# joesound212985/Deepfake-Detection-using-CLIP-Based-SigLIP-2-Vision-Transformers

Hardware: AMD Instinct MI355X
Metric: images/sec (train fwd+bwd) SigLIP-2-so400m@384 bf16 (higher is better)
Workload: dtype bf16; 1 GPU; so400m-patch14-384 encoder+pool-head train fwd+bwd, 384x384, per-GPU batch 128, seeded random weights; global_batch=128, parallelism=dp1

## Files before the change

deepfake-detection-using-clip-based-siglip-2-vision-transformers_amd/csrc/encoder.hip:

```cpp
#include <hip/hip_runtime.h>
#include <string.h>

#include <algorithm>
#include <new>
#include <vector>

#include "kernels.h"
#include "siglip_hip.h"

using namespace sgl;

namespace {

inline size_t align256(size_t x) { return (x + 255) & ~(size_t)255; }
inline char* at(void* base, size_t off) { return reinterpret_cast<char*>(base) + off; }
inline const char* at(const void* base, size_t off) { return reinterpret_cast<const char*>(base) + off; }
inline bool mfma16(int dt) { return dt == DT_BF16 || dt == DT_F16; }
inline int round_up(int x, int m) { return (x + m - 1) / m * m; }

struct Bump {
  size_t off = 0;
  size_t take(size_t bytes) {
    const size_t o = off;
    off += align256(bytes);
    return o;
  }
};

struct ShadowLayer {
  size_t wqkv, wqkv_t, wo, wo_t, w1, w1_t, w2, w2_t, bqkv, b1;
  size_t wqkv_s, wo_s, w1_s, w2_s;
};

}

struct sgl_ctx {
  sgl_config cfg;
  int D, I, Ip, L, H, dh, DP, P, K0, Kp, g0, dt;
  size_t es;
  int split = 0;
  int mx = 0;
  int Dp = 0;
  int recompute = 0;
  int last_hip = 0;
  size_t sh_wpatch = 0;
  std::vector<ShadowLayer> sh_layers;
  size_t sh_hwkv = 0, sh_hwkv_t = 0, sh_hwo = 0, sh_hwo_t = 0, sh_hw1 = 0, sh_hw1_t = 0, sh_hw2 = 0, sh_hw2_t = 0,
         sh_hb1 = 0;
  size_t sh_total = 0;
};

namespace {

constexpr int kMaxLayers = 128;

constexpr size_t kSplitWsBytes = (size_t)256 * 256 * 256 * 4;

inline size_t head_bytes(const sgl_ctx* c, int B, int N) { return (size_t)B * c->H * N * c->DP * c->es; }

struct Layout {
  int B = 0, gh = 0, gw = 0, N = 0, M = 0;
  bool train = false;
  size_t a_im2col = 0, a_pos = 0;
  size_t a_layer0 = 0, a_layer_stride = 0;
  size_t r_stats1 = 0, r_h1 = 0, r_qkv = 0, r_attn = 0, r_lse = 0, r_xmid = 0, r_stats2 = 0, r_h2 = 0, r_u = 0, r_a = 0,
         r_attq = 0;
  size_t a_pstats = 0, a_lastlp = 0, a_kvh = 0, a_qp = 0, a_probs = 0, a_ao = 0, a_h0 = 0, a_hstats = 0, a_hl = 0, a_hu = 0,
         a_ha = 0;
  size_t a_spa = 0, a_spb = 0, w_spa = 0, w_spb = 0;
  size_t act_total = 0;
  size_t w_dx = 0, w_g = 0, w_du = 0, w_dh = 0, w_dqkv = 0, w_delta = 0, w_splitws = 0, w_lnpart = 0, w_cspart = 0,
         w_dlast = 0, w_gsum = 0, w_csum = 0;
  size_t w_hg = 0, w_hdu = 0, w_hdh = 0, w_hdao = 0, w_hdqpart = 0, w_hdqp = 0, w_hdh0 = 0;
  size_t ws_bwd_total = 0;
  size_t saved_total = 0, ws_total = 0, ws_act_off = 0;
  bool rc = false;
  size_t w_blk = 0;

  Layout() = default;
  Layout(const sgl_ctx* c, int B_, int Himg, int Wimg, bool train_) {
    B = B_;
    train = train_;
    rc = train && c->recompute;
    gh = Himg / c->P;
    gw = Wimg / c->P;
    N = gh * gw;
    M = B * N;
    const size_t es = c->es, D = c->D, Ip = c->Ip, Mz = (size_t)M;
    Bump a;
    a_im2col = a.take(Mz * c->Kp * es);
    a_pos = a.take((size_t)N * D * 4);
    Bump r;
    const size_t Dp = c->Dp;
    const bool mx = c->mx;
    r_stats1 = r.take(Mz * 2 * 4);
    r_h1 = r.take(mx ? Mz * Dp + Mz * Dp / 32 : Mz * D * es);
    r_qkv = r.take(3 * head_bytes(c, B, N));
    r_attn = r.take(Mz * D * es);
    r_lse = r.take((size_t)B * c->H * N * 4);
    r_xmid = r.take(Mz * D * 4);
    r_stats2 = r.take(Mz * 2 * 4);
    r_h2 = r.take(mx ? Mz * Dp + Mz * Dp / 32 : Mz * D * es);
    r_u = r.take(mx ? 0 : Mz * Ip * es);
    r_a = r.take(mx ? Mz * Ip + Mz * Ip / 32 : Mz * Ip * es);
    r_attq = r.take(mx ? Mz * Dp + Mz * Dp / 32 : 0);
    a_layer_stride = (train && !rc) ? r.off : 0;
    a_layer0 = a.take(rc ? 0 : train ? r.off * (size_t)c->L : r.off);
    a_pstats = a.take(Mz * 2 * 4);
    a_lastlp = a.take(Mz * D * es);
// ... 1303 lines not shown
```

deepfake-detection-using-clip-based-siglip-2-vision-transformers_amd/csrc/gemm_bf16.hip:

```cpp
#include <stdlib.h>

#include "common.hip.h"
#include "epilogue.hip.h"
#include "kernels.h"

namespace sgl {

constexpr int G_BM = 128, G_BN = 128, G_BK = 64;
constexpr int G_STAGE = (G_BM + G_BN) * G_BK * 2;
constexpr int G_CT_LD = 132;
constexpr int G_LDS = (2 * G_STAGE > G_BM * G_CT_LD * 4) ? 2 * G_STAGE : G_BM * G_CT_LD * 4;

__device__ __forceinline__ u32x4 ldg128(__amdgpu_buffer_rsrc_t r, uint32_t voff) {
  return __builtin_amdgcn_raw_buffer_load_b128(r, voff, 0, 0);
}

template <int EPI, typename TOut>
__device__ __forceinline__ void store_tile(char* smem, f32x4 (&acc)[4][4], int wr, int wc, int lane, int t, int m0,
                                           int n0, int M, int N, const EpiParams& p) {
  float* ct = reinterpret_cast<float*>(smem);
  __syncthreads();
  const int g = lane >> 4, c16 = lane & 15;
#pragma unroll
  for (int i = 0; i < 4; ++i)
// ... 217 lines not shown
#pragma unroll
      for (int i = 0; i < 4; ++i)
#pragma unroll
        for (int j = 0; j < 4; ++j)
          acc[i][j] = mfma_16x16x32(af[i], bfr[j], acc[i][j]);
    }
    if (kt + 1 < nk) store_stage(cur ^ 1);
    __syncthreads();
  }
  EpiParams pq = p;
  if (p.split_stride) pq.out = reinterpret_cast<float*>(p.out) + (size_t)blockIdx.y * p.split_stride;
  store_tile<EPI_F32, float>(smem, acc, wr, wc, lane, t, n1_0, n2_0, N1, N2, pq);
}

template <int EPI, typename TOut, typename TIn>
static hipError_t launch_nt(const TIn* A, int lda, const TIn* B, int ldb, int M, int N, int K, const EpiParams& p,
                            hipStream_t s) {
  const hipError_t e = set_max_dynamic_lds_once<&gemm_nt_kernel<EPI, TOut, TIn>>(G_LDS);
  if (e != hipSuccess) return e;
  const int tiles = ((M + G_BM - 1) / G_BM) * ((N + G_BN - 1) / G_BN);
  hipLaunchKernelGGL((gemm_nt_kernel<EPI, TOut, TIn>), dim3(tiles), dim3(256), G_LDS, s, A, lda, B, ldb, M, N, K, p);
  return hipGetLastError();
}

template <typename TIn>
static hipError_t gemm_nt_mfma(const void* A, int lda, const void* B, int ldb, int M, int N, int K, int epi,
                               int out_dtype, const EpiParams& p, hipStream_t s) {
  if (M == 0 || N == 0) return hipSuccess;
  if ((lda % 8) || (ldb % 8) || (K % 8) || K <= 0) return hipErrorInvalidValue;
  if (epi != EPI_F32 && (N % 8)) return hipErrorInvalidValue;
  if ((size_t)M * lda * 2 >= (1ull << 32) || (size_t)N * ldb * 2 >= (1ull << 32)) return hipErrorInvalidValue;
  if (M >= 2048 && N >= 256) {
    static const int tile_env = getenv("SGL_NT_TILE") ? atoi(getenv("SGL_NT_TILE")) : 0;
    const bool can384 = epi == EPI_STORE || epi == EPI_RES_F32;
    const bool pays384 = N % 192 == 0 && N % 256 != 0 && (epi == EPI_STORE || K >= 2048);
    const bool want384 = tile_env == 384 || (tile_env != 256 && pays384);
    if (can384 && want384) return gemm_nt384<TIn>(A, lda, B, ldb, M, N, K, epi, out_dtype, p, s);
    return gemm_nt256<TIn>(A, lda, B, ldb, M, N, K, epi, out_dtype, p, s);
  }
  return dispatch_epilogue<TIn>(epi, out_dtype, [&](auto tag) {
    using T = decltype(tag);
    return launch_nt<T::epi, typename T::out, TIn>((const TIn*)A, lda, (const TIn*)B, ldb, M, N, K, p, s);
  });
}
hipError_t gemm_nt_bf16(const void* A, int lda, const void* B, int ldb, int M, int N, int K, int epi, int out_dtype,
                        const EpiParams& p, hipStream_t s) {
  return gemm_nt_mfma<bf16>(A, lda, B, ldb, M, N, K, epi, out_dtype, p, s);
}
hipError_t gemm_nt_f16(const void* A, int lda, const void* B, int ldb, int M, int N, int K, int epi, int out_dtype,
                       const EpiParams& p, hipStream_t s) {
  return gemm_nt_mfma<f16>(A, lda, B, ldb, M, N, K, epi, out_dtype, p, s);
}

template <typename Launch>
static hipError_t tn_split_k(int Mred, int N1, int N2, int splits, const EpiParams& p_, hipStream_t s, float* split_ws,
                             size_t split_ws_bytes, Launch&& launch) {
  EpiParams p = p_;
  float* out = reinterpret_cast<float*>(p.out);
  if (splits < 1) splits = 1;
  int m_per = (Mred + splits - 1) / splits;
  m_per = ((m_per + G_BK - 1) / G_BK) * G_BK;
  splits = (Mred + m_per - 1) / m_per;
  if (splits > 1) {
    const size_t slab = (size_t)N1 * N2;
    if (split_ws && (size_t)splits * slab * sizeof(float) <= split_ws_bytes && p.alpha == 1.0f && !p.bias &&
        (N2 % 4 == 0) && (p.ldo % 4 == 0) && ((((uintptr_t)out) | ((uintptr_t)split_ws)) & 15) == 0) {
      EpiParams q = p;
      q.out = split_ws;
      q.ldo = N2;
      q.accumulate = 0;
      q.atomic = 0;
      q.split_stride = slab;
      const hipError_t e = launch(m_per, splits, q);
      if (e != hipSuccess) return e;
      return reduce_splits(split_ws, splits, slab, N1, N2, out, p.ldo, p.accumulate, s);
    }
    if (!p.accumulate) {
      const hipError_t e = hipMemset2DAsync(out, (size_t)p.ldo * sizeof(float), 0, (size_t)N2 * sizeof(float), N1, s);
      if (e != hipSuccess) return e;
    }
    p.atomic = 1;
  }
  return launch(m_per, splits, p);
}

template <typename TIn>
static hipError_t gemm_tn_mfma(const void* A, int lda, const void* B, int ldb, int Mred, int N1, int N2, int splits,
                               const EpiParams& p, hipStream_t s, float* split_ws, size_t split_ws_bytes) {
  if (N1 == 0 || N2 == 0) return hipSuccess;
  if ((lda % 8) || (ldb % 8)) return hipErrorInvalidValue;
  if ((size_t)Mred * lda * 2 >= (1ull << 32) || (size_t)Mred * ldb * 2 >= (1ull << 32)) return hipErrorInvalidValue;
  if (Mred <= 0) {
    if (!p.accumulate)
      return hipMemset2DAsync(p.out, (size_t)p.ldo * sizeof(float), 0, (size_t)N2 * sizeof(float), N1, s);
    return hipSuccess;
  }
  if (N1 >= 512 && N2 >= 512 && Mred >= 2048) {
    const int tiles = ((N1 + 255) / 256) * ((N2 + 255) / 256);
    int sp = 256 / tiles;
    if (sp < 1) sp = 1;
    const int max_sp = Mred / 1024 > 0 ? Mred / 1024 : 1;
    if (sp > max_sp) sp = max_sp;
    return tn_split_k(Mred, N1, N2, sp, p, s, split_ws, split_ws_bytes, [&](int m_per, int nsplit, const EpiParams& q) {
      return gemm_tn256<TIn>(A, lda, B, ldb, Mred, N1, N2, m_per, nsplit, q, s);
    });
  }
  return tn_split_k(Mred, N1, N2, splits, p, s, split_ws, split_ws_bytes, [&](int m_per, int nsplit, const EpiParams& q) {
    const hipError_t e = set_max_dynamic_lds_once<&gemm_tn_kernel<TIn>>(G_LDS);
    if (e != hipSuccess) return e;
    const int tiles = ((N1 + G_BM - 1) / G_BM) * ((N2 + G_BN - 1) / G_BN);
    hipLaunchKernelGGL(gemm_tn_kernel<TIn>, dim3(tiles, nsplit), dim3(256), G_LDS, s, (const TIn*)A, lda, (const TIn*)B,
                       ldb, Mred, N1, N2, m_per, q);
    return hipGetLastError();
  });
}
hipError_t gemm_tn_bf16(const void* A, int lda, const void* B, int ldb, int Mred, int N1, int N2, int splits,
                        const EpiParams& p, hipStream_t s, float* split_ws, size_t split_ws_bytes) {
  return gemm_tn_mfma<bf16>(A, lda, B, ldb, Mred, N1, N2, splits, p, s, split_ws, split_ws_bytes);
}
hipError_t gemm_tn_f16(const void* A, int lda, const void* B, int ldb, int Mred, int N1, int N2, int splits,
                       const EpiParams& p, hipStream_t s, float* split_ws, size_t split_ws_bytes) {
  return gemm_tn_mfma<f16>(A, lda, B, ldb, Mred, N1, N2, splits, p, s, split_ws, split_ws_bytes);
}

}
```

deepfake-detection-using-clip-based-siglip-2-vision-transformers_amd/csrc/gemm_bf16_v2.hip:

```cpp
#include <stdlib.h>
#ifdef SGL_TIMELINE
#include <stdio.h>
#include <string.h>
#endif

#include "common.hip.h"
#include "epilogue.hip.h"
#include "kernels.h"

namespace sgl {

constexpr int T_BK = 64;

template <int BM_, int BN_, int MI_, int MJ_>
struct NtTileShape {
  static constexpr int BM = BM_, BN = BN_, MI = MI_, MJ = MJ_;
  static constexpr int WM = 16 * MI, WN = 16 * MJ;
  static constexpr int NWR = BM / WM, NWC = BN / WN;
  static constexpr int OPA = BM * T_BK * 2;
  static constexpr int STAGE = (BM + BN) * T_BK * 2;
  static constexpr int LDS = 2 * STAGE;
  static constexpr int PA = BM / 128, PB = BN / 64, NI = 2 * PA + PB;
  static constexpr int CT_LD = BN + 4;
  static_assert(NWR * WM == BM && NWC * WN == BN && NWR * NWC == 8, "8 waves = 512 threads cover the tile");
  static_assert(MI % 2 == 0 && BM % 128 == 0 && BN % 64 == 0 && 64 % NWR == 0 && (64 / NWR) % 16 == 0, "halves, pieces, passes");
  static_assert(LDS <= 160 * 1024 && 64 * CT_LD * 4 <= LDS, "two stages, and the epilogue image, in 160 KiB of LDS");
};

struct NtTile256 : NtTileShape<256, 256, 8, 4> {
  static __device__ __forceinline__ int wr(int w) { return (w >> 1) & 1; }
  static __device__ __forceinline__ int wc(int w) { return (w & 1) + 2 * (w >> 2); }
  static __device__ __forceinline__ int b_row(int w, int q) {
    const int ul = 16 * w + 8 * (q & 1);
    return (ul >> 5) * 64 + (ul & 31) + 32 * (q >> 1);
  }
  static constexpr bool takes(int epi) { return true; }
};

struct NtTile384 : NtTileShape<384, 192, 6, 6> {
  static __device__ __forceinline__ int wr(int w) { return w & 3; }
  static __device__ __forceinline__ int wc(int w) { return w >> 2; }
  static __device__ __forceinline__ int b_row(int w, int q) { return 8 * (3 * w + q); }
  static constexpr bool takes(int epi) { return epi == EPI_STORE || epi == EPI_RES_F32; }
};

constexpr int gcd_of(int a, int b) { return b == 0 ? a : gcd_of(b, a % b); }

template <typename G, int EPI, typename TOut>
__device__ __forceinline__ void store_tile_pp(char* smem, f32x4 (&acc)[G::MI][G::MJ], int wr, int wc, int lane, int t,
                                              int m0, int n0, int M, int N, const EpiParams& p) {
  static_assert(G::takes(EPI), "this tile geometry is not dispatched with this epilogue");
  float* ct = reinterpret_cast<float*>(smem);
  const int g = lane >> 4, c16 = lane & 15;
  constexpr int NV = (sizeof(TOut) == 4) ? 4 : 8;
  constexpr int CT_LD = G::CT_LD;
  constexpr int CPR = G::BN / NV;
  constexpr int WR_ROWS = 64 / G::NWR;
  constexpr int BLK = WR_ROWS / 16;
  constexpr int NPASS = G::BM / 64;
  constexpr int QN = (64 * CPR) / 512;
  constexpr int P = CPR / gcd_of(CPR, 512);
  static_assert(NPASS * BLK == G::MI && (64 * CPR) % 512 == 0 && (512 * P) % CPR == 0, "staging image and chunk walk");
  auto grow_of = [&](int pass, int row) { return m0 + (row / WR_ROWS) * G::WM + pass * WR_ROWS + row % WR_ROWS; };
  constexpr bool HAS_BIAS = (EPI == EPI_BIAS_GELU || EPI == EPI_RES_F32 || EPI == EPI_QKV);
  int tcol[P], gcol[P];
  bool col_ok[P];
  float bias[P][NV];
  size_t qkv_c0[P];
  int qkv_pad[P];
#pragma unroll
  for (int h = 0; h < P; ++h) {
    tcol[h] = ((t + 512 * h) % CPR) * NV;
    gcol[h] = n0 + tcol[h];
    col_ok[h] = gcol[h] < N;
#pragma unroll
    for (int j = 0; j < NV; ++j) bias[h][j] = 0.f;
    if constexpr (HAS_BIAS) {
      if (col_ok[h]) Vec<float, NV>::ld(p.bias + gcol[h], bias[h]);
    }
    qkv_c0[h] = 0;
    qkv_pad[h] = 0;
    if constexpr (EPI == EPI_QKV) {
      const int dm = p.heads * p.head_dim;
      const int which = gcol[h] / dm;
      const int hc = gcol[h] - which * dm;
      const int hd = hc / p.head_dim;
      const int d = hc - hd * p.head_dim;
      qkv_c0[h] = ((size_t)which * p.batch * p.heads + hd) * (size_t)p.tokens * p.head_dim_pad + d;
      qkv_pad[h] = (d + NV == p.head_dim) ? (p.head_dim_pad - p.head_dim) / NV : 0;
    }
  }
  float csum[NV];
#pragma unroll
  for (int j = 0; j < NV; ++j) csum[j] = 0.f;
  using PreT = u32x4;
  constexpr bool HAS_PRE = (EPI == EPI_RES_F32 || EPI == EPI_GELU_BWD);
// ... 73 lines not shown
            for (int j = 0; j < NV; ++j) u[j] = (float)ub[j];
          } else {
            const f32x4 uf = __builtin_bit_cast(f32x4, pre[pass & 1][q]);
#pragma unroll
            for (int j = 0; j < NV; ++j) u[j] = uf[j];
          }
          epi_gelu_bwd<TOut, NV>(p, v, u, reinterpret_cast<TOut*>(p.out) + (size_t)grow * p.ldo + gcol[h]);
#pragma unroll
          for (int j = 0; j < NV; ++j) csum[j] += v[j];
        } else {
          epi_apply<EPI, TOut, NV>(p, grow, gcol[h], N, v);
        }
      }
    }
  }
  if constexpr (EPI == EPI_GELU_BWD) {
    static_assert(P == 1, "the bias-gradient fold needs one column set per thread");
    epi_colsum_fold<512, G::BN, NV>(ct, csum, t, m0, n0, N, p);
  }
}

__device__ __forceinline__ int unit_of_block(int bid, int per) { return (bid & 7) * per + (bid >> 3); }

__device__ __forceinline__ void tile_of_unit(int u, int tiles_m, int tiles_n, int& tile_m, int& tile_n, int bh = 8) {
  const int band = u / (bh * tiles_n);
  const int rows = (tiles_m - band * bh < bh) ? tiles_m - band * bh : bh;
  const int r = u - band * bh * tiles_n;
  tile_n = r / rows;
  tile_m = band * bh + (r - tile_n * rows);
}

__device__ __forceinline__ bool tile_of_local(int xcd, int v, int tiles_m, int tiles_n, int cgw, int& tm, int& tn) {
  const int r_lo = (xcd * tiles_m) >> 3, r_hi = ((xcd + 1) * tiles_m) >> 3;
  const int R = r_hi - r_lo;
  if (v >= R * tiles_n) return false;
  const int full = R * cgw;
  const int g = v / full, rem = v - g * full;
  const int w = (tiles_n - g * cgw < cgw) ? tiles_n - g * cgw : cgw;
  const int r = rem / w;
  tm = r_lo + r;
  tn = g * cgw + (rem - r * w);
  return true;
}

__device__ __forceinline__ void pp_dma16(u32x4 desc, uint32_t lds_addr, uint32_t voff) {
  asm volatile("s_mov_b32 m0, %0\n\ts_nop 0\n\tbuffer_load_dwordx4 %1, %2, 0 offen lds"
               :: "s"(lds_addr), "v"(voff), "s"(desc) : "memory");
}
__device__ __forceinline__ u32x4 pp_desc(const void* base, uint32_t bytes) {
  const uint64_t q = (uint64_t)base;
  u32x4 d = {(uint32_t)q, (uint32_t)(q >> 32) & 0xffffu, bytes, 0x00020000u};
  return d;
}
template <int NI>
__device__ __forceinline__ void pp_end_read() {
  asm volatile("s_waitcnt vmcnt(%0) lgkmcnt(0)" :: "n"(NI) : "memory");
  __builtin_amdgcn_sched_barrier(0);
  __builtin_amdgcn_s_barrier();
  __builtin_amdgcn_sched_barrier(0);
}
#define SGL_PP_END_MFMA()                 \
  do {                                    \
    __builtin_amdgcn_sched_barrier(0);    \
    __builtin_amdgcn_s_barrier();         \
    __builtin_amdgcn_sched_barrier(0);    \
  } while (0)

#ifdef SGL_TIMELINE
__device__ unsigned long long g_nt6_tl[4];
__device__ unsigned long long g_tn6_tl[12];
#define SGL_TL_STAMP(v) const unsigned long long v = __builtin_readcyclecounter()
#else
#define SGL_TL_STAMP(v)
#endif

template <typename G, int EPI, typename TOut, typename TIn>
__global__ __launch_bounds__(512, 2) void gemm_nt6_kernel(const TIn* __restrict__ A, int lda,
                                                          const TIn* __restrict__ B, int ldb, int M, int N, int K,
                                                          int tiles_m, int tiles_n, int band_h, EpiParams p) {
  extern __shared__ __attribute__((aligned(16))) char smem[];
  SGL_TL_STAMP(tl0);
  const int ntiles = tiles_m * tiles_n;
  int tile_m, tile_n;
  if (band_h < 0) {
    if (!tile_of_local(blockIdx.x & 7, blockIdx.x >> 3, tiles_m, tiles_n, -band_h, tile_m, tile_n)) return;
  } else {
    const int unit = unit_of_block(blockIdx.x, (ntiles + 7) >> 3);
    if (unit >= ntiles) return;
    tile_of_unit(unit, tiles_m, tiles_n, tile_m, tile_n, band_h);
  }
  constexpr int MI = G::MI, MJ = G::MJ, HI = MI / 2, PA = G::PA, PB = G::PB, NI = G::NI;
  const int t = threadIdx.x, lane = t & 63;
  const int w = __builtin_amdgcn_readfirstlane(t >> 6);
  const int wr = G::wr(w), wc = G::wc(w), grp = w >> 2;
  const int m0 = tile_m * G::BM, n0 = tile_n * G::BN;
  const int rows_a = (M - m0 < G::BM) ? M - m0 : G::BM;
  const int rows_b = (N - n0 < G::BN) ? N - n0 : G::BN;
  const u32x4 da = pp_desc(A + (size_t)m0 * lda, (uint32_t)(((size_t)(rows_a - 1) * lda + K) * 2));
  const u32x4 db = pp_desc(B + (size_t)n0 * ldb, (uint32_t)(((size_t)(rows_b - 1) * ldb + K) * 2));
  const uint32_t lds0 = (uint32_t)(size_t)((SGL_LDS char*)smem);

  enum { U_A0 = 0, U_B = 1, U_A1 = 2 };
  constexpr int PMAX = PA > PB ? PA : PB;
  const int drow = lane >> 3, dchunk = (lane & 7) ^ drow;
  uint32_t voff[3][PMAX], ldst[3][PMAX];
#pragma unroll
// ... 38 lines not shown
  lo_x8<TIn> fa[2 * HI], fb[2 * MJ];
  auto mfma_slot = [&](int i0) {
    if (active) {
      __builtin_amdgcn_s_setprio(1);
#pragma unroll
      for (int h = 0; h < 2; ++h)
#pragma unroll
        for (int i = 0; i < HI; ++i)
#pragma unroll
          for (int j = 0; j < MJ; ++j)
            acc[i0 + i][j] = mfma_16x16x32(fa[HI * h + i], fb[MJ * h + j], acc[i0 + i][j]);
      __builtin_amdgcn_s_setprio(0);
    }
    SGL_PP_END_MFMA();
  };
  for (int kt = 0; kt < nk; ++kt) {
    const char* base = smem + (kt & 1) * G::STAGE;
    const char* pa = base + fa_base;
    const char* pb = base + fb_base;
    if (active) {
#pragma unroll
      for (int f = 0; f < 2 * MJ; ++f) fb[f] = *reinterpret_cast<const lo_x8<TIn>*>(pb + (f % MJ) * 2048 + ((f / MJ) ? c1 : c0));
#pragma unroll
      for (int f = 0; f < 2 * HI; ++f) fa[f] = *reinterpret_cast<const lo_x8<TIn>*>(pa + (f % HI) * 2048 + ((f / HI) ? c1 : c0));
    }
    issue(U_A1, kt + 1);
    pp_end_read<NI>();
    mfma_slot(0);
    if (active) {
#pragma unroll
      for (int f = 0; f < 2 * HI; ++f) fa[f] = *reinterpret_cast<const lo_x8<TIn>*>(pa + (HI + f % HI) * 2048 + ((f / HI) ? c1 : c0));
    }
    issue(U_A0, kt + 2); issue(U_B, kt + 2);
    pp_end_read<NI>();
    mfma_slot(HI);
  }
  if (grp == 0) SGL_PP_END_MFMA();
  asm volatile("s_waitcnt vmcnt(0)" ::: "memory");
#ifdef SGL_TIMELINE
  if (p.atomic == 77) return;
#endif
  SGL_TL_STAMP(tl1);
  store_tile_pp<G, EPI, TOut>(smem, acc, wr, wc, lane, t, m0, n0, M, N, p);
#ifdef SGL_TIMELINE
  SGL_TL_STAMP(tl2);
  if (t == 0) {
    atomicAdd(&g_nt6_tl[0], tl1 - tl0);
    atomicAdd(&g_nt6_tl[1], tl2 - tl1);
    atomicAdd(&g_nt6_tl[2], 1ull);
  }
#endif
}

template <typename TIn>
__global__ __launch_bounds__(512, 2) void gemm_tn6_kernel(const TIn* __restrict__ A, int lda,
                                                          const TIn* __restrict__ B, int ldb, int Mred, int N1, int N2,
                                                          int m_per_split, int nsplits, int tiles_1, int tiles_2,
                                                          EpiParams p) {
  using G = NtTile256;
  extern __shared__ __attribute__((aligned(16))) char smem[];
  const int ntiles = tiles_1 * tiles_2;
  const int nunits = ntiles * nsplits;
  const int unit = unit_of_block(blockIdx.x, (nunits + 7) >> 3);
  if (unit >= nunits) return;
  const int split = unit / ntiles, trem = unit - split * ntiles;
  const int tile1 = trem / tiles_2, tile2 = trem - tile1 * tiles_2;
  const int t = threadIdx.x, lane = t & 63;
  const int w = __builtin_amdgcn_readfirstlane(t >> 6);
  const int wr = G::wr(w), wc = G::wc(w), grp = w >> 2;
  const int n1_0 = tile1 * G::BM, n2_0 = tile2 * G::BN;
  const int m_begin = split * m_per_split;
  const int m_end = (m_begin + m_per_split < Mred) ? m_begin + m_per_split : Mred;
  const int rows = m_end - m_begin;
  const u32x4 da = pp_desc(A + (size_t)m_begin * lda, (uint32_t)((size_t)rows * lda * 2));
  const u32x4 db = pp_desc(B + (size_t)m_begin * ldb, (uint32_t)((size_t)rows * ldb * 2));
  const uint32_t lds0 = (uint32_t)(size_t)((SGL_LDS char*)smem);

  const int dr2 = lane >> 5, dslot = lane & 31;
  uint32_t voff[4][2], ldst[4][2];
#pragma unroll
  for (int u = 0; u < 4; ++u)
#pragma unroll
    for (int q = 0; q < 2; ++q) {
      const int r0 = 32 * (u >> 1) + 4 * w + 2 * q;
      const int row = r0 + dr2;
      const int chunk = dslot ^ (2 * (row & 3) + 8 * ((row >> 3) & 1));
      const bool isA = (u & 1) == 0;
      const int col = (isA ? n1_0 : n2_0) + chunk * 8;
      const int lim = isA ? N1 : N2;
      const int ld = isA ? lda : ldb;
      voff[u][q] = (col < lim) ? (uint32_t)(row * ld + col) * 2u : SGL_OOB;
      ldst[u][q] = lds0 + (isA ? 0 : G::OPA) + (uint32_t)r0 * 512u;
    }
  auto issue = [&](int u, int kt) {
    const uint32_t r0 = (uint32_t)kt * T_BK;
    const uint32_t sb = (uint32_t)((kt & 1) * G::STAGE);
    const bool isA = (u & 1) == 0;
    const u32x4 d = isA ? da : db;
    const uint32_t adv = r0 * (uint32_t)(isA ? lda : ldb) * 2u;
#pragma unroll
    for (int q = 0; q < 2; ++q) pp_dma16(d, ldst[u][q] + sb, voff[u][q] == SGL_OOB ? SGL_OOB : voff[u][q] + adv);
  };

  const int fg = lane >> 4, fq = (lane >> 2) & 3, fp = lane & 3;
  const uint32_t swz = (uint32_t)(32 * fq + 128 * (fg & 1));
  const uint32_t frow = (uint32_t)((8 * fg + fq) * 512);
  const uint32_t fa_col = ((uint32_t)(wr * 256 + 8 * fp)) ^ swz;
  const uint32_t fb_col = ((uint32_t)(wc * 128 + 8 * fp)) ^ swz;
  const bool active = (n2_0 + wc * G::WN < N2) && (n1_0 + wr * G::WM < N1);

  f32x4 acc[G::MI][G::MJ];
#pragma unroll
  for (int i = 0; i < 8; ++i)
#pragma unroll
    for (int j = 0; j < 4; ++j) acc[i][j] = f32x4{0.f, 0.f, 0.f, 0.f};

  const int nk = (rows + T_BK - 1) / T_BK;
  issue(0, 0); issue(1, 0); issue(2, 0); issue(3, 0);
  issue(0, 1); issue(1, 1);
  pp_end_read<8>();
  if (grp == 1) SGL_PP_END_MFMA();

#define SGL_TR6(ptr) \
  __builtin_shufflevector(lds_read_tr16<TIn>(ptr), lds_read_tr16<TIn>((ptr) + 4 * 512), 0, 1, 2, 3, 4, 5, 6, 7)
  lo_x8<TIn> fa[8], fb[4];
#ifdef SGL_TIMELINE
  unsigned long long tlp[5] = {0, 0, 0, 0, 0};
#define SGL_TLP(i) do { const unsigned long long n_ = __builtin_readcyclecounter(); tlp[i] += n_ - tl_last; tl_last = n_; } while (0)
  unsigned long long tl_last = __builtin_readcyclecounter();
#else
#define SGL_TLP(i)
#endif
  for (int kt = 0; kt < nk; ++kt) {
    const char* base = smem + (kt & 1) * G::STAGE + frow;
#pragma unroll
    for (int h = 0; h < 2; ++h) {
      if (active) {
#pragma unroll
        for (int j = 0; j < 4; ++j) fb[j] = SGL_TR6(base + G::OPA + h * 32 * 512 + (fb_col ^ (uint32_t)(j * 32)));
#pragma unroll
        for (int i = 0; i < 8; ++i) fa[i] = SGL_TR6(base + h * 32 * 512 + (fa_col ^ (uint32_t)(i * 32)));
      }
      if (h == 0) { issue(2, kt + 1); issue(3, kt + 1); }
      else { issue(0, kt + 2); issue(1, kt + 2); }
#ifdef SGL_TIMELINE
      SGL_TLP(0);
      asm volatile("s_waitcnt vmcnt(8) lgkmcnt(0)" ::: "memory");
      SGL_TLP(1);
      __builtin_amdgcn_sched_barrier(0);
      __builtin_amdgcn_s_barrier();
      __builtin_amdgcn_sched_barrier(0);
      SGL_TLP(2);
#else
      pp_end_read<8>();
#endif
      if (active) {
        __builtin_amdgcn_s_setprio(1);
#pragma unroll
        for (int i = 0; i < 8; ++i)
#pragma unroll
          for (int j = 0; j < 4; ++j)
            acc[i][j] = mfma_16x16x32(fa[i], fb[j], acc[i][j]);
        __builtin_amdgcn_s_setprio(0);
      }
#ifdef SGL_TIMELINE
      asm volatile("s_nop 0" ::"v"(acc[0][0]), "v"(acc[7][3]));
      SGL_TLP(3);
#endif
      SGL_PP_END_MFMA();
      SGL_TLP(4);
    }
  }
#ifdef SGL_TIMELINE
  if (lane == 0 && active && (w == 0 || w == 4)) {
    for (int i = 0; i < 5; ++i) atomicAdd(&g_tn6_tl[(w >> 2) * 6 + i], tlp[i]);
    atomicAdd(&g_tn6_tl[(w >> 2) * 6 + 5], (unsigned long long)(2 * nk));
  }
#endif
#undef SGL_TR6
  if (grp == 0) SGL_PP_END_MFMA();
  asm volatile("s_waitcnt vmcnt(0)" ::: "memory");
  EpiParams pq = p;
  if (p.split_stride) pq.out = reinterpret_cast<float*>(p.out) + (size_t)split * p.split_stride;
  store_tile_pp<G, EPI_F32, float>(smem, acc, wr, wc, lane, t, n1_0, n2_0, N1, N2, pq);
}

#ifdef SGL_TIMELINE
template <int NC, typename Print>
static void timeline_report(hipStream_t s, unsigned long long (&counters)[NC], Print&& print) {
  if (!getenv("SGL_TIMELINE")) return;
  unsigned long long h[NC];
  (void)hipStreamSynchronize(s);
  (void)hipMemcpyFromSymbol(h, HIP_SYMBOL(counters), sizeof(h));
  print(h);
  memset(h, 0, sizeof(h));
  (void)hipMemcpyToSymbol(HIP_SYMBOL(counters), h, sizeof(h));
}
#endif

template <typename G, int EPI, typename TOut, typename TIn>
static hipError_t launch_nt_pp(const TIn* A, int lda, const TIn* B, int ldb, int M, int N, int K, const EpiParams& p,
                               hipStream_t s) {
  const hipError_t e = set_max_dynamic_lds_once<&gemm_nt6_kernel<G, EPI, TOut, TIn>>(G::LDS);
  if (e != hipSuccess) return e;
  const int tiles_m = (M + G::BM - 1) / G::BM, tiles_n = (N + G::BN - 1) / G::BN;
  static const int band_env = getenv("SGL_BAND") ? atoi(getenv("SGL_BAND")) : 0;
  const int band_h = band_env != 0 ? band_env : -8;
  const int grid = band_h < 0 ? 8 * (((tiles_m + 7) / 8) * tiles_n)
                              : ((tiles_m * tiles_n + 7) / 8) * 8;
  EpiParams pp = p;
#ifdef SGL_TIMELINE
  static const bool skip_epi = getenv("SGL_NT6_SKIP_EPI") != nullptr;
  if (skip_epi && EPI != EPI_F32) pp.atomic = 77;
#endif
  hipLaunchKernelGGL((gemm_nt6_kernel<G, EPI, TOut, TIn>), dim3(grid), dim3(512), G::LDS, s, A, lda, B, ldb, M, N, K,
                     tiles_m, tiles_n, band_h, pp);
#ifdef SGL_TIMELINE
  timeline_report(s, g_nt6_tl, [&](const unsigned long long* h) {
    if (h[2])
      fprintf(stderr, "[timeline] gemm_nt6 %dx%d EPI %d M=%d N=%d K=%d: %llu tiles, main loop %.0f, epilogue %.0f cycles per tile\n",
              G::BM, G::BN, EPI, M, N, K, h[2], (double)h[0] / h[2], (double)h[1] / h[2]);
  });
#endif
  return hipGetLastError();
}

template <typename G, typename TIn>
static hipError_t gemm_nt_pp(const void* A, int lda, const void* B, int ldb, int M, int N, int K, int epi, int out_dtype,
                             const EpiParams& p, hipStream_t s) {
  return dispatch_epilogue<TIn>(epi, out_dtype, [&](auto tag) {
    using T = decltype(tag);
    if constexpr (G::takes(T::epi))
      return launch_nt_pp<G, T::epi, typename T::out, TIn>((const TIn*)A, lda, (const TIn*)B, ldb, M, N, K, p, s);
    else
      return hipErrorInvalidValue;
  });
}
template <typename TIn>
hipError_t gemm_nt256(const void* A, int lda, const void* B, int ldb, int M, int N, int K, int epi, int out_dtype,
                      const EpiParams& p, hipStream_t s) {
  return gemm_nt_pp<NtTile256, TIn>(A, lda, B, ldb, M, N, K, epi, out_dtype, p, s);
}
template <typename TIn>
hipError_t gemm_nt384(const void* A, int lda, const void* B, int ldb, int M, int N, int K, int epi, int out_dtype,
                      const EpiParams& p, hipStream_t s) {
  return gemm_nt_pp<NtTile384, TIn>(A, lda, B, ldb, M, N, K, epi, out_dtype, p, s);
}

template <typename TIn>
hipError_t gemm_tn256(const void* A, int lda, const void* B, int ldb, int Mred, int N1, int N2, int m_per, int splits,
                      const EpiParams& p, hipStream_t s) {
  using G = NtTile256;
  const hipError_t e = set_max_dynamic_lds_once<&gemm_tn6_kernel<TIn>>(G::LDS);
  if (e != hipSuccess) return e;
  const int tiles_1 = (N1 + G::BM - 1) / G::BM, tiles_2 = (N2 + G::BN - 1) / G::BN;
  const int grid = ((tiles_1 * tiles_2 * splits + 7) / 8) * 8;
  hipLaunchKernelGGL(gemm_tn6_kernel<TIn>, dim3(grid), dim3(512), G::LDS, s, (const TIn*)A, lda, (const TIn*)B, ldb, Mred,
                     N1, N2, m_per, splits, tiles_1, tiles_2, p);
#ifdef SGL_TIMELINE
  timeline_report(s, g_tn6_tl, [&](const unsigned long long* h) {
    for (int g = 0; g < 2; ++g)
      if (h[g * 6 + 5])
        fprintf(stderr, "[timeline] gemm_tn6 N1=%d N2=%d Mred=%d splits=%d group %d, cycles per slot pair (read slot + MFMA slot): issue "
                "reads+DMA %.0f, wait %.0f, barrier %.0f, 32 MFMAs %.0f, barrier %.0f\n", N1, N2, Mred, splits, g,
                (double)h[g * 6 + 0] / h[g * 6 + 5], (double)h[g * 6 + 1] / h[g * 6 + 5], (double)h[g * 6 + 2] / h[g * 6 + 5],
                (double)h[g * 6 + 3] / h[g * 6 + 5], (double)h[g * 6 + 4] / h[g * 6 + 5]);
  });
#endif
  return hipGetLastError();
}

#define SGL_INSTANTIATE_PP(TIn)                                                                                        \
  template hipError_t gemm_nt256<TIn>(const void*, int, const void*, int, int, int, int, int, int, const EpiParams&,   \
                                      hipStream_t);                                                                    \
  template hipError_t gemm_nt384<TIn>(const void*, int, const void*, int, int, int, int, int, int, const EpiParams&,   \
                                      hipStream_t);                                                                    \
  template hipError_t gemm_tn256<TIn>(const void*, int, const void*, int, int, int, int, int, int, const EpiParams&,   \
                                      hipStream_t);
SGL_INSTANTIATE_PP(bf16)
SGL_INSTANTIATE_PP(f16)
#undef SGL_INSTANTIATE_PP

}
```

deepfake-detection-using-clip-based-siglip-2-vision-transformers_amd/csrc/kernels.h:

```cpp
#pragma once
#include <hip/hip_runtime.h>
#include <stddef.h>
#include <stdint.h>

#include "siglip_hip.h"

namespace sgl {

enum DType : int {
  DT_F32 = 0,
  DT_BF16 = 1,
  DT_F32_MFMA = 2,
  DT_F16 = 3,
};
static inline size_t dtype_size(int dt) { return (dt == DT_BF16 || dt == DT_F16) ? 2 : 4; }

template <auto Kernel>
hipError_t set_max_dynamic_lds_once(int bytes) {
  static bool done = false;
  if (done) return hipSuccess;
  const hipError_t e =
      hipFuncSetAttribute(reinterpret_cast<const void*>(Kernel), hipFuncAttributeMaxDynamicSharedMemorySize, bytes);
  done = e == hipSuccess;
  return e;
// ... 68 lines not shown
};
void cast_job_add(CastJob& job, const float* src, int R, int C, int lds_, void* dst, int Rp, int Cp, int ldd, void* dst_t,
                  int ldt);
void cast_job_add_vec(CastJob& job, const float* src, int n, float* dst, int np);
hipError_t cast_job_run(const CastJob& job, int dst_dtype, hipStream_t s);
hipError_t split3_rows(const float* src, int R, int C, int ld, void* dst, int Cs, int b_side, hipStream_t s);
hipError_t split3_stack(const float* src, int R, int C, int ld, void* dst, int Cs, int b_side, hipStream_t s);
int colsum_chunks(int M);
hipError_t colsum(const void* in, int dtype, int ld, int M, int N, int n_out, float* partial ,
                  float* out, int accumulate, hipStream_t s);
hipError_t batch_sum(const float* in, int B, size_t n, float* out, int accumulate, hipStream_t s);
hipError_t vecmat_f32(const float* v, const float* W, int rows, int cols, float* scratch, float* out, int accumulate,
                      hipStream_t s);
hipError_t pos_resize(const float* table, int g0, float* out, int gh, int gw, int D, hipStream_t s);
hipError_t pos_resize_bwd(const float* dout, int gh, int gw, float* dtable, int g0, int D, hipStream_t s);
hipError_t copy_f32(const float* src, float* dst, size_t n, hipStream_t s);
hipError_t cast_f32(const float* src, void* dst, int dst_dtype, size_t n, hipStream_t s);
hipError_t add_f32(const float* a, const float* b, float* out, size_t n, hipStream_t s);
static inline size_t pool_attn_lds_floats(int N, int DP, int backward) {
  const size_t part = (size_t)N * (DP / 8) > (size_t)256 * 8 ? (size_t)N * (DP / 8) : (size_t)256 * 8;
  return part + (backward ? 2 : 1) * (size_t)N + 8;
}
static inline int pool_attn_max_tokens(int DP, int backward) {
  return (int)((64 * 1024 / sizeof(float) - 8) / (size_t)(DP / 8 + (backward ? 2 : 1)));
}
hipError_t pool_attn_fwd(const float* q, const void* K, const void* V, int dtype, void* out ,
                         float* probs , int B, int H, int N, int dh, int DP, hipStream_t s);
hipError_t pool_attn_bwd(const float* q, const void* K, const void* V, int dtype, const float* probs,
                         const float* dout , void* dkv ,
                         float* dq_partial , int B, int H, int N, int dh, int DP, hipStream_t s);

hipError_t gemm_f32_generic(const float* A, long sam, long sak, const float* B, long sbn, long sbk, int M, int N,
                            int K, int epi, int out_dtype, const EpiParams& p, hipStream_t s);

hipError_t gemm_nt_bf16(const void* A, int lda, const void* B, int ldb, int M, int N, int K, int epi,
                        int out_dtype, const EpiParams& p, hipStream_t s);
hipError_t reduce_splits(const float* ws, int splits, size_t stride, int N1, int N2, float* out, int ldo, int accumulate,
                         hipStream_t s);
hipError_t gemm_tn_bf16(const void* A, int lda, const void* B, int ldb, int Mred, int N1, int N2, int splits,
                        const EpiParams& p, hipStream_t s, float* split_ws = nullptr, size_t split_ws_bytes = 0);
hipError_t gemm_nt_f16(const void* A, int lda, const void* B, int ldb, int M, int N, int K, int epi, int out_dtype,
                       const EpiParams& p, hipStream_t s);
hipError_t gemm_tn_f16(const void* A, int lda, const void* B, int ldb, int Mred, int N1, int N2, int splits,
                       const EpiParams& p, hipStream_t s, float* split_ws = nullptr, size_t split_ws_bytes = 0);
template <typename TIn>
hipError_t gemm_nt256(const void* A, int lda, const void* B, int ldb, int M, int N, int K, int epi, int out_dtype,
                      const EpiParams& p, hipStream_t s);
template <typename TIn>
hipError_t gemm_nt384(const void* A, int lda, const void* B, int ldb, int M, int N, int K, int epi, int out_dtype,
                      const EpiParams& p, hipStream_t s);
template <typename TIn>
hipError_t gemm_tn256(const void* A, int lda, const void* B, int ldb, int Mred, int N1, int N2, int m_per, int splits,
                      const EpiParams& p, hipStream_t s);

hipError_t attn_fwd(const void* q, const void* k, const void* v, int dtype, void* out, float* lse, int B, int H,
                    int N, int dh, int DP, int ld_qkv, hipStream_t s);
hipError_t attn_bwd(const void* q, const void* k, const void* v, const void* out, const void* dout,
                    const float* lse, int dtype, void* dqkv, float* delta, float* reserved, int B, int H, int N,
                    int dh, int DP, int ld_qkv, hipStream_t s);

}
```

Before: 430.4 images/sec.

## Add 384x192 TN weight-gradient tile with cost-model split planner

Generalizes the TN (weight-gradient) pipelined kernel over tile shape and adds a 384x192 variant. A constexpr planner picks tile and split-K count by minimizing per-CU work, given the available split workspace. It also moves buffer descriptors into scalar registers via readfirstlane and lets the 384 NT tile take the f32 epilogue. The aim is better CU balance and less wave quantization for out_proj and QKV dW GEMMs. The trade-off is a more complex load distribution, where one extra B piece is issued by a wave group, plus more code paths.

```diff
diff --git a/deepfake-detection-using-clip-based-siglip-2-vision-transformers_amd/csrc/encoder.hip b/deepfake-detection-using-clip-based-siglip-2-vision-transformers_amd/csrc/encoder.hip
--- a/deepfake-detection-using-clip-based-siglip-2-vision-transformers_amd/csrc/encoder.hip
+++ b/deepfake-detection-using-clip-based-siglip-2-vision-transformers_amd/csrc/encoder.hip
@@ -55,6 +55,8 @@
 constexpr int kMaxLayers = 128;
 
 constexpr size_t kSplitWsBytes = (size_t)256 * 256 * 256 * 4;
+static_assert(tn_plan_is(93312, 1152, 1152, kSplitWsBytes, 384, 12), "out_proj dW in the encoder's workspace");
+static_assert(tn_plan_is(93312, 3456, 1152, kSplitWsBytes, 384, 4), "QKV dW in the encoder's workspace");
 
 inline size_t head_bytes(const sgl_ctx* c, int B, int N) { return (size_t)B * c->H * N * c->DP * c->es; }
 
diff --git a/deepfake-detection-using-clip-based-siglip-2-vision-transformers_amd/csrc/gemm_bf16.hip b/deepfake-detection-using-clip-based-siglip-2-vision-transformers_amd/csrc/gemm_bf16.hip
--- a/deepfake-detection-using-clip-based-siglip-2-vision-transformers_amd/csrc/gemm_bf16.hip
+++ b/deepfake-detection-using-clip-based-siglip-2-vision-transformers_amd/csrc/gemm_bf16.hip
@@ -293,6 +293,11 @@
   return gemm_nt_mfma<f16>(A, lda, B, ldb, M, N, K, epi, out_dtype, p, s);
 }
 
+static bool tn_slabs_ok(const EpiParams& p, int N2, const float* split_ws) {
+  return p.alpha == 1.0f && !p.bias && (N2 % 4 == 0) && (p.ldo % 4 == 0) &&
+         ((((uintptr_t)p.out) | ((uintptr_t)split_ws)) & 15) == 0;
+}
+
 template <typename Launch>
 static hipError_t tn_split_k(int Mred, int N1, int N2, int splits, const EpiParams& p_, hipStream_t s, float* split_ws,
                              size_t split_ws_bytes, Launch&& launch) {
@@ -304,8 +309,7 @@
   splits = (Mred + m_per - 1) / m_per;
   if (splits > 1) {
     const size_t slab = (size_t)N1 * N2;
-    if (split_ws && (size_t)splits * slab * sizeof(float) <= split_ws_bytes && p.alpha == 1.0f && !p.bias &&
-        (N2 % 4 == 0) && (p.ldo % 4 == 0) && ((((uintptr_t)out) | ((uintptr_t)split_ws)) & 15) == 0) {
+    if (split_ws && (size_t)splits * slab * sizeof(float) <= split_ws_bytes && tn_slabs_ok(p, N2, split_ws)) {
       EpiParams q = p;
       q.out = split_ws;
       q.ldo = N2;
@@ -337,12 +341,13 @@
     return hipSuccess;
   }
   if (N1 >= 512 && N2 >= 512 && Mred >= 2048) {
-    const int tiles = ((N1 + 255) / 256) * ((N2 + 255) / 256);
-    int sp = 256 / tiles;
-    if (sp < 1) sp = 1;
-    const int max_sp = Mred / 1024 > 0 ? Mred / 1024 : 1;
-    if (sp > max_sp) sp = max_sp;
-    return tn_split_k(Mred, N1, N2, sp, p, s, split_ws, split_ws_bytes, [&](int m_per, int nsplit, const EpiParams& q) {
+    static const int tile_env = getenv("SGL_TN_TILE") ? atoi(getenv("SGL_TN_TILE")) : 0;
+    const int tile = (tile_env == 256 || tile_env == 384) ? tile_env : 0;
+    const bool slabs_ok = split_ws && tn_slabs_ok(p, N2, split_ws);
+    TnPlan plan = tn_plan(Mred, N1, N2, slabs_ok ? split_ws_bytes : 0, tile);
+    if (plan.splits == 1) plan = tn_plan(Mred, N1, N2, ~(size_t)0, tile);
+    return tn_split_k(Mred, N1, N2, plan.splits, p, s, split_ws, split_ws_bytes, [&](int m_per, int nsplit, const EpiParams& q) {
+      if (plan.tile == 384) return gemm_tn384<TIn>(A, lda, B, ldb, Mred, N1, N2, m_per, nsplit, q, s);
       return gemm_tn256<TIn>(A, lda, B, ldb, Mred, N1, N2, m_per, nsplit, q, s);
     });
   }
diff --git a/deepfake-detection-using-clip-based-siglip-2-vision-transformers_amd/csrc/gemm_bf16_v2.hip b/deepfake-detection-using-clip-based-siglip-2-vision-transformers_amd/csrc/gemm_bf16_v2.hip
--- a/deepfake-detection-using-clip-based-siglip-2-vision-transformers_amd/csrc/gemm_bf16_v2.hip
+++ b/deepfake-detection-using-clip-based-siglip-2-vision-transformers_amd/csrc/gemm_bf16_v2.hip
@@ -41,7 +41,7 @@
   static __device__ __forceinline__ int wr(int w) { return w & 3; }
   static __device__ __forceinline__ int wc(int w) { return w >> 2; }
   static __device__ __forceinline__ int b_row(int w, int q) { return 8 * (3 * w + q); }
-  static constexpr bool takes(int epi) { return epi == EPI_STORE || epi == EPI_RES_F32; }
+  static constexpr bool takes(int epi) { return epi == EPI_STORE || epi == EPI_RES_F32 || epi == EPI_F32; }
 };
 
 constexpr int gcd_of(int a, int b) { return b == 0 ? a : gcd_of(b, a % b); }
@@ -221,6 +221,10 @@
   u32x4 d = {(uint32_t)q, (uint32_t)(q >> 32) & 0xffffu, bytes, 0x00020000u};
   return d;
 }
+__device__ __forceinline__ u32x4 pp_desc_sgpr(u32x4 d) {
+  return u32x4{(uint32_t)__builtin_amdgcn_readfirstlane((int)d[0]), (uint32_t)__builtin_amdgcn_readfirstlane((int)d[1]),
+               (uint32_t)__builtin_amdgcn_readfirstlane((int)d[2]), (uint32_t)__builtin_amdgcn_readfirstlane((int)d[3])};
+}
 template <int NI>
 __device__ __forceinline__ void pp_end_read() {
   asm volatile("s_waitcnt vmcnt(%0) lgkmcnt(0)" :: "n"(NI) : "memory");
@@ -365,13 +369,26 @@
 #endif
 }
 
-template <typename TIn>
+template <int ROWB>
+__device__ __forceinline__ int tn_swz(int m) {
+  static_assert(ROWB % 128 == 0, "the patterns are closed inside 256 / 128 bytes of a row");
+  if constexpr (ROWB % 256 == 0) return 2 * (m & 3) + 8 * ((m >> 3) & 1);
+  else return 2 * ((m >> 1) & 1) + 4 * ((m >> 3) & 1);
+}
+
+template <typename G, typename TIn>
 __global__ __launch_bounds__(512, 2) void gemm_tn6_kernel(const TIn* __restrict__ A, int lda,
                                                           const TIn* __restrict__ B, int ldb, int Mred, int N1, int N2,
                                                           int m_per_split, int nsplits, int tiles_1, int tiles_2,
                                                           EpiParams p) {
-  using G = NtTile256;
   extern __shared__ __attribute__((aligned(16))) char smem[];
+  constexpr int MI = G::MI, MJ = G::MJ;
+  constexpr int RA = 2 * G::BM, RB = 2 * G::BN;
+  constexpr int HA = G::BM / 16, HB = G::BN / 16;
+  constexpr int PA = HA / 8, PB = HB / 8;
+  constexpr bool BX = (HB % 8) != 0;
+  constexpr int NI = 2 * PA + 2 * PB + (BX ? 1 : 0);
+  static_assert(HA % 8 == 0 && (HB % 8 == 0 || HB % 8 == 4), "pieces of a k-half over 8 waves (+ one wave group)");
   const int ntiles = tiles_1 * tiles_2;
   const int nunits = ntiles * nsplits;
   const int unit = unit_of_block(blockIdx.x, (nunits + 7) >> 3);
@@ -385,58 +402,69 @@
   const int m_begin = split * m_per_split;
   const int m_end = (m_begin + m_per_split < Mred) ? m_begin + m_per_split : Mred;
   const int rows = m_end - m_begin;
-  const u32x4 da = pp_desc(A + (size_t)m_begin * lda, (uint32_t)((size_t)rows * lda * 2));
-  const u32x4 db = pp_desc(B + (size_t)m_begin * ldb, (uint32_t)((size_t)rows * ldb * 2));
+  const u32x4 da = pp_desc_sgpr(pp_desc(A + (size_t)m_begin * lda, (uint32_t)((size_t)rows * lda * 2)));
+  const u32x4 db = pp_desc_sgpr(pp_desc(B + (size_t)m_begin * ldb, (uint32_t)((size_t)rows * ldb * 2)));
   const uint32_t lds0 = (uint32_t)(size_t)((SGL_LDS char*)smem);
 
-  const int dr2 = lane >> 5, dslot = lane & 31;
-  uint32_t voff[4][2], ldst[4][2];
-#pragma unroll
-  for (int u = 0; u < 4; ++u)
-#pragma unroll
-    for (int q = 0; q < 2; ++q) {
-      const int r0 = 32 * (u >> 1) + 4 * w + 2 * q;
-      const int row = r0 + dr2;
-      const int chunk = dslot ^ (2 * (row & 3) + 8 * ((row >> 3) & 1));
-      const bool isA = (u & 1) == 0;
-      const int col = (isA ? n1_0 : n2_0) + chunk * 8;
-      const int lim = isA ? N1 : N2;
-      const int ld = isA ? lda : ldb;
-      voff[u][q] = (col < lim) ? (uint32_t)(row * ld + col) * 2u : SGL_OOB;
-      ldst[u][q] = lds0 + (isA ? 0 : G::OPA) + (uint32_t)r0 * 512u;
-    }
-  auto issue = [&](int u, int kt) {
+  uint32_t voffA[2][PA], ldsA[2][PA], voffB[2][PB + 1], ldsB[2][PB + 1];
+#pragma unroll
+  for (int h = 0; h < 2; ++h) {
+#pragma unroll
+    for (int q = 0; q < PA; ++q) {
+      const int piece = PA * w + q, pos = 1024 * piece + 16 * lane;
+      const int row = 32 * h + pos / RA, chunk = ((pos % RA) >> 4) ^ tn_swz<RA>(row);
+      const int col = n1_0 + chunk * 8;
+      voffA[h][q] = (col < N1) ? (uint32_t)(row * lda + col) * 2u : SGL_OOB;
+      ldsA[h][q] = lds0 + (uint32_t)(h * 32 * RA + 1024 * piece);
+    }
+#pragma unroll
+    for (int q = 0; q < PB + 1; ++q) {
+      const int piece = (q < PB) ? PB * w + q : 8 * PB + (w & 3), pos = 1024 * piece + 16 * lane;
+      const int row = 32 * h + pos / RB, chunk = ((pos % RB) >> 4) ^ tn_swz<RB>(row);
+      const int col = n2_0 + chunk * 8;
+      voffB[h][q] = (col < N2) ? (uint32_t)(row * ldb + col) * 2u : SGL_OOB;
+      ldsB[h][q] = lds0 + (uint32_t)(G::OPA + h * 32 * RB + 1024 * piece);
+    }
+  }
+  auto issue = [&](int h, int kt) {
     const uint32_t r0 = (uint32_t)kt * T_BK;
     const uint32_t sb = (uint32_t)((kt & 1) * G::STAGE);
-    const bool isA = (u & 1) == 0;
-    const u32x4 d = isA ? da : db;
-    const uint32_t adv = r0 * (uint32_t)(isA ? lda : ldb) * 2u;
-#pragma unroll
-    for (int q = 0; q < 2; ++q) pp_dma16(d, ldst[u][q] + sb, voff[u][q] == SGL_OOB ? SGL_OOB : voff[u][q] + adv);
+    const uint32_t adva = r0 * (uint32_t)lda * 2u, advb = r0 * (uint32_t)ldb * 2u;
+#pragma unroll
+    for (int q = 0; q < PA; ++q) pp_dma16(da, ldsA[h][q] + sb, voffA[h][q] == SGL_OOB ? SGL_OOB : voffA[h][q] + adva);
+#pragma unroll
+    for (int q = 0; q < PB; ++q) pp_dma16(db, ldsB[h][q] + sb, voffB[h][q] == SGL_OOB ? SGL_OOB : voffB[h][q] + advb);
+    if constexpr (BX) {
+      if (grp == h) pp_dma16(db, ldsB[h][PB] + sb, voffB[h][PB] == SGL_OOB ? SGL_OOB : voffB[h][PB] + advb);
+    }
   };
 
   const int fg = lane >> 4, fq = (lane >> 2) & 3, fp = lane & 3;
-  const uint32_t swz = (uint32_t)(32 * fq + 128 * (fg & 1));
-  const uint32_t frow = (uint32_t)((8 * fg + fq) * 512);
-  const uint32_t fa_col = ((uint32_t)(wr * 256 + 8 * fp)) ^ swz;
-  const uint32_t fb_col = ((uint32_t)(wc * 128 + 8 * fp)) ^ swz;
+  const int fm = 8 * fg + fq;
+  uint32_t fa_off[MI], fb_off[MJ];
+#pragma unroll
+  for (int i = 0; i < MI; ++i)
+    fa_off[i] = (uint32_t)(fm * RA) + ((uint32_t)(wr * G::WM * 2 + i * 32 + 8 * fp) ^ (uint32_t)(16 * tn_swz<RA>(fm)));
+#pragma unroll
+  for (int j = 0; j < MJ; ++j)
+    fb_off[j] = (uint32_t)(G::OPA + fm * RB) + ((uint32_t)(wc * G::WN * 2 + j * 32 + 8 * fp) ^ (uint32_t)(16 * tn_swz<RB>(fm)));
   const bool active = (n2_0 + wc * G::WN < N2) && (n1_0 + wr * G::WM < N1);
 
-  f32x4 acc[G::MI][G::MJ];
-#pragma unroll
-  for (int i = 0; i < 8; ++i)
-#pragma unroll
-    for (int j = 0; j < 4; ++j) acc[i][j] = f32x4{0.f, 0.f, 0.f, 0.f};
+  f32x4 acc[MI][MJ];
+#pragma unroll
+  for (int i = 0; i < MI; ++i)
+#pragma unroll
+    for (int j = 0; j < MJ; ++j) acc[i][j] = f32x4{0.f, 0.f, 0.f, 0.f};
 
   const int nk = (rows + T_BK - 1) / T_BK;
-  issue(0, 0); issue(1, 0); issue(2, 0); issue(3, 0);
-  issue(0, 1); issue(1, 1);
-  pp_end_read<8>();
+  issue(0, 0); issue(1, 0);
+  issue(0, 1);
+  pp_end_read<NI>();
   if (grp == 1) SGL_PP_END_MFMA();
 
-#define SGL_TR6(ptr) \
-  __builtin_shufflevector(lds_read_tr16<TIn>(ptr), lds_read_tr16<TIn>((ptr) + 4 * 512), 0, 1, 2, 3, 4, 5, 6, 7)
-  lo_x8<TIn> fa[8], fb[4];
+#define SGL_TR6(ptr, rowb) \
+  __builtin_shufflevector(lds_read_tr16<TIn>(ptr), lds_read_tr16<TIn>((ptr) + 4 * (rowb)), 0, 1, 2, 3, 4, 5, 6, 7)
+  lo_x8<TIn> fa[MI], fb[MJ];
 #ifdef SGL_TIMELINE
   unsigned long long tlp[5] = {0, 0, 0, 0, 0};
 #define SGL_TLP(i) do { const unsigned long long n_ = __builtin_readcyclecounter(); tlp[i] += n_ - tl_last; tl_last = n_; } while (0)
@@ -445,39 +473,39 @@
 #define SGL_TLP(i)
 #endif
   for (int kt = 0; kt < nk; ++kt) {
-    const char* base = smem + (kt & 1) * G::STAGE + frow;
+    const char* base = smem + (kt & 1) * G::STAGE;
 #pragma unroll
     for (int h = 0; h < 2; ++h) {
       if (active) {
 #pragma unroll
-        for (int j = 0; j < 4; ++j) fb[j] = SGL_TR6(base + G::OPA + h * 32 * 512 + (fb_col ^ (uint32_t)(j * 32)));
-#pragma unroll
-        for (int i = 0; i < 8; ++i) fa[i] = SGL_TR6(base + h * 32 * 512 + (fa_col ^ (uint32_t)(i * 32)));
+        for (int j = 0; j < MJ; ++j) fb[j] = SGL_TR6(base + h * 32 * RB + fb_off[j], RB);
+#pragma unroll
+        for (int i = 0; i < MI; ++i) fa[i] = SGL_TR6(base + h * 32 * RA + fa_off[i], RA);
       }
-      if (h == 0) { issue(2, kt + 1); issue(3, kt + 1); }
-      else { issue(0, kt + 2); issue(1, kt + 2); }
+      if (h == 0) issue(1, kt + 1);
+      else issue(0, kt + 2);
 #ifdef SGL_TIMELINE
       SGL_TLP(0);
-      asm volatile("s_waitcnt vmcnt(8) lgkmcnt(0)" ::: "memory");
+      asm volatile("s_waitcnt vmcnt(%0) lgkmcnt(0)" :: "n"(NI) : "memory");
       SGL_TLP(1);
       __builtin_amdgcn_sched_barrier(0);
       __builtin_amdgcn_s_barrier();
       __builtin_amdgcn_sched_barrier(0);
       SGL_TLP(2);
 #else
-      pp_end_read<8>();
+      pp_end_read<NI>();
 #endif
       if (active) {
         __builtin_amdgcn_s_setprio(1);
 #pragma unroll
-        for (int i = 0; i < 8; ++i)
-#pragma unroll
-          for (int j = 0; j < 4; ++j)
+        for (int i = 0; i < MI; ++i)
+#pragma unroll
+          for (int j = 0; j < MJ; ++j)
             acc[i][j] = mfma_16x16x32(fa[i], fb[j], acc[i][j]);
         __builtin_amdgcn_s_setprio(0);
       }
 #ifdef SGL_TIMELINE
-      asm volatile("s_nop 0" ::"v"(acc[0][0]), "v"(acc[7][3]));
+      asm volatile("s_nop 0" ::"v"(acc[0][0]), "v"(acc[MI - 1][MJ - 1]));
       SGL_TLP(3);
 #endif
       SGL_PP_END_MFMA();
@@ -560,27 +588,36 @@
   return gemm_nt_pp<NtTile384, TIn>(A, lda, B, ldb, M, N, K, epi, out_dtype, p, s);
 }
 
+template <typename G, typename TIn>
+static hipError_t launch_tn_pp(const void* A, int lda, const void* B, int ldb, int Mred, int N1, int N2, int m_per,
+                               int splits, const EpiParams& p, hipStream_t s) {
+  const hipError_t e = set_max_dynamic_lds_once<&gemm_tn6_kernel<G, TIn>>(G::LDS);
+  if (e != hipSuccess) return e;
+  const int tiles_1 = (N1 + G::BM - 1) / G::BM, tiles_2 = (N2 + G::BN - 1) / G::BN;
+  const int grid = ((tiles_1 * tiles_2 * splits + 7) / 8) * 8;
+  hipLaunchKernelGGL((gemm_tn6_kernel<G, TIn>), dim3(grid), dim3(512), G::LDS, s, (const TIn*)A, lda, (const TIn*)B, ldb,
+                     Mred, N1, N2, m_per, splits, tiles_1, tiles_2, p);
+#ifdef SGL_TIMELINE
+  timeline_report(s, g_tn6_tl, [&](const unsigned long long* h) {
+    for (int g = 0; g < 2; ++g)
+      if (h[g * 6 + 5])
+        fprintf(stderr, "[timeline] gemm_tn6 %dx%d N1=%d N2=%d Mred=%d splits=%d group %d, cycles per slot pair (read slot + MFMA slot): "
+                "issue reads+DMA %.0f, wait %.0f, barrier %.0f, %d MFMAs %.0f, barrier %.0f\n", G::BM, G::BN, N1, N2, Mred, splits, g,
+                (double)h[g * 6 + 0] / h[g * 6 + 5], (double)h[g * 6 + 1] / h[g * 6 + 5], (double)h[g * 6 + 2] / h[g * 6 + 5],
+                G::MI * G::MJ, (double)h[g * 6 + 3] / h[g * 6 + 5], (double)h[g * 6 + 4] / h[g * 6 + 5]);
+  });
+#endif
+  return hipGetLastError();
+}
 template <typename TIn>
 hipError_t gemm_tn256(const void* A, int lda, const void* B, int ldb, int Mred, int N1, int N2, int m_per, int splits,
                       const EpiParams& p, hipStream_t s) {
-  using G = NtTile256;
-  const hipError_t e = set_max_dynamic_lds_once<&gemm_tn6_kernel<TIn>>(G::LDS);
-  if (e != hipSuccess) return e;
-  const int tiles_1 = (N1 + G::BM - 1) / G::BM, tiles_2 = (N2 + G::BN - 1) / G::BN;
-  const int grid = ((tiles_1 * tiles_2 * splits + 7) / 8) * 8;
-  hipLaunchKernelGGL(gemm_tn6_kernel<TIn>, dim3(grid), dim3(512), G::LDS, s, (const TIn*)A, lda, (const TIn*)B, ldb, Mred,
-                     N1, N2, m_per, splits, tiles_1, tiles_2, p);
-#ifdef SGL_TIMELINE
-  timeline_report(s, g_tn6_tl, [&](const unsigned long long* h) {
-    for (int g = 0; g < 2; ++g)
-      if (h[g * 6 + 5])
-        fprintf(stderr, "[timeline] gemm_tn6 N1=%d N2=%d Mred=%d splits=%d group %d, cycles per slot pair (read slot + MFMA slot): issue "
-                "reads+DMA %.0f, wait %.0f, barrier %.0f, 32 MFMAs %.0f, barrier %.0f\n", N1, N2, Mred, splits, g,
-                (double)h[g * 6 + 0] / h[g * 6 + 5], (double)h[g * 6 + 1] / h[g * 6 + 5], (double)h[g * 6 + 2] / h[g * 6 + 5],
-                (double)h[g * 6 + 3] / h[g * 6 + 5], (double)h[g * 6 + 4] / h[g * 6 + 5]);
-  });
-#endif
-  return hipGetLastError();
+  return launch_tn_pp<NtTile256, TIn>(A, lda, B, ldb, Mred, N1, N2, m_per, splits, p, s);
+}
+template <typename TIn>
+hipError_t gemm_tn384(const void* A, int lda, const void* B, int ldb, int Mred, int N1, int N2, int m_per, int splits,
+                      const EpiParams& p, hipStream_t s) {
+  return launch_tn_pp<NtTile384, TIn>(A, lda, B, ldb, Mred, N1, N2, m_per, splits, p, s);
 }
 
 #define SGL_INSTANTIATE_PP(TIn)                                                                                        \
@@ -589,6 +626,8 @@
   template hipError_t gemm_nt384<TIn>(const void*, int, const void*, int, int, int, int, int, int, const EpiParams&,   \
                                       hipStream_t);                                                                    \
   template hipError_t gemm_tn256<TIn>(const void*, int, const void*, int, int, int, int, int, int, const EpiParams&,   \
+                                      hipStream_t);                                                                    \
+  template hipError_t gemm_tn384<TIn>(const void*, int, const void*, int, int, int, int, int, int, const EpiParams&,   \
                                       hipStream_t);
 SGL_INSTANTIATE_PP(bf16)
 SGL_INSTANTIATE_PP(f16)
diff --git a/deepfake-detection-using-clip-based-siglip-2-vision-transformers_amd/csrc/kernels.h b/deepfake-detection-using-clip-based-siglip-2-vision-transformers_amd/csrc/kernels.h
--- a/deepfake-detection-using-clip-based-siglip-2-vision-transformers_amd/csrc/kernels.h
+++ b/deepfake-detection-using-clip-based-siglip-2-vision-transformers_amd/csrc/kernels.h
@@ -144,6 +144,43 @@
 template <typename TIn>
 hipError_t gemm_tn256(const void* A, int lda, const void* B, int ldb, int Mred, int N1, int N2, int m_per, int splits,
                       const EpiParams& p, hipStream_t s);
+template <typename TIn>
+hipError_t gemm_tn384(const void* A, int lda, const void* B, int ldb, int Mred, int N1, int N2, int m_per, int splits,
+                      const EpiParams& p, hipStream_t s);
+
+struct TnPlan {
+  int tile, splits, m_per;
+};
+constexpr TnPlan tn_plan(int Mred, int N1, int N2, size_t ws_bytes, int tile = 0) {
+  TnPlan best = {0, 0, 0};
+  long best_cost = 0;
+  for (int g = 0; g < 2; ++g) {
+    const int bm = g ? 384 : 256, bn = g ? 192 : 256, area8 = g ? 9 : 8;
+    if (tile != 0 && tile != bm) continue;
+    const int tiles = ((N1 + bm - 1) / bm) * ((N2 + bn - 1) / bn);
+    for (int sp = 1; sp == 1 || (tiles * sp <= 256 && Mred / sp >= 1024); ++sp) {
+      if (sp > 1 && (size_t)sp * N1 * N2 * sizeof(float) > ws_bytes) break;
+      const int m_per = ((Mred + sp - 1) / sp + 63) / 64 * 64;
+      const long cost = (long)area8 * m_per;
+      if (best.tile == 0 || cost < best_cost) {
+        best = {bm, (Mred + m_per - 1) / m_per, m_per};
+        best_cost = cost;
+      }
+    }
+  }
+  return best;
+}
+constexpr bool tn_plan_is(int Mred, int N1, int N2, size_t ws_bytes, int tile, int splits) {
+  const TnPlan p = tn_plan(Mred, N1, N2, ws_bytes);
+  return (tile == 0 || p.tile == tile) && p.splits == splits;
+}
+constexpr size_t kTnSlabBytes = (size_t)256 * 384 * 192 * 4;
+static_assert(tn_plan_is(93312, 1152, 1152, kTnSlabBytes, 384, 14), "out_proj dW");
+static_assert(tn_plan_is(93312, 3456, 1152, kTnSlabBytes, 384, 4), "QKV dW");
+static_assert(tn_plan_is(93312, 4304, 1152, kTnSlabBytes, 256, 3), "fc1 dW");
+static_assert(tn_plan_is(93312, 1152, 4304, kTnSlabBytes, 256, 3), "fc2 dW");
+static_assert(tn_plan_is(4133, 520, 1152, kTnSlabBytes, 0, 4) && tn_plan(4133, 520, 1152, kTnSlabBytes).m_per == 1088, "digest case");
+static_assert(tn_plan_is(2048, 512, 512, kTnSlabBytes, 256, 2) && tn_plan(2048, 512, 512, kTnSlabBytes).m_per == 1024, "digest case");
 
 hipError_t attn_fwd(const void* q, const void* k, const void* v, int dtype, void* out, float* lse, int B, int H,
                     int N, int dh, int DP, int ld_qkv, hipStream_t s);
```

Result: faster. 435.5 images/sec (median of 6 runs) (+1.2%).
